# menyifang/MIMO

Measured on NVIDIA H100. Metric: frames/sec @ 512x512x24f, 20 DDIM steps, higher is better.
Workload: dtype fp16

## Files before the change

### mimo_b200/csrc/gemm_wgmma.cu

```cuda
#include <cuda_runtime.h>

#include <cudaTypedefs.h>

#include "../../include/mimo_b200.h"
#include "host_util.h"
#include "ptx.cuh"
#include "wgmma.cuh"

namespace mimo {

constexpr int BM = 128;
constexpr int BK = 64;
constexpr int kGemmThreads = 320;
constexpr int kChunk = 8192;

struct EpiArgs {
  const void* bias;
  const void* rowvec;
  long long rows_per_group;
  long long ld_rowvec;
  float scale;
  int act;
  float* partial;
};

struct ConvGeom {
  int conv;
  int H, W, NI;
  int TW, TH, TN;
  int tiles_w, tiles_h;
  int ctot;
  int c0;
  int kb0, kb1;
  int a_bytes;
  int chunk_bytes;
  int splits;
  int kb_split;
  int ntaps;
  signed char tdx[9], tdy[9];
};

template <int BN, bool kRes>
struct GemmCfg {
  static constexpr int kStageBytes = BM * BK * 2 + BN * BK * 2;
  static constexpr int kNChunk = BN / 32;
  static constexpr int kOutBytes = 2 * kChunk;
  static constexpr int kResSlots = kRes ? 2 : 0;
  static constexpr int kResBytes = kResSlots * kChunk;
  static constexpr int kBarBytes = 512;
  static constexpr int kFixed = kBarBytes + 2048  + kOutBytes + kResBytes;
  static constexpr int kMaxStages = (BN >= 256) ? 4 : (BN >= 160 ? 5 : (BN >= 128 ? 6 : 8));
  static constexpr int kFit = (227 * 1024 - kFixed) / kStageBytes;
  static constexpr int kStages = kFit < kMaxStages ? kFit : kMaxStages;
  static constexpr int kSmemBytes = kStages * kStageBytes + kFixed;
  static_assert(kStages >= 3, "pipeline too shallow");
};

template <int BN, bool kBf16, bool kRes>
__global__ void __launch_bounds__(kGemmThreads, 1)
gemm_wgmma_kernel(const __grid_constant__ CUtensorMap tmA0, const __grid_constant__ CUtensorMap tmA1,
                  const __grid_constant__ CUtensorMap tmB, const __grid_constant__ CUtensorMap tmOut,
                  const __grid_constant__ CUtensorMap tmRes, int M, int N, int num_m_tiles, int num_n_tiles,
                  int num_k_blocks, ConvGeom g, EpiArgs ep) {
  using Cfg = GemmCfg<BN, kRes>;
  using C = Cvt<kBf16>;
  using T = typename C::T;
  constexpr int NCHUNK = Cfg::kNChunk;
  extern __shared__ __align__(1024) uint8_t smem[];
  uint8_t* sOut = smem + Cfg::kStages * Cfg::kStageBytes;
  uint8_t* sRes = sOut + Cfg::kOutBytes;
  uint64_t* bars = reinterpret_cast<uint64_t*>(sRes + Cfg::kResBytes);
  uint64_t* full_bar = bars;
  uint64_t* empty_bar = bars + 8;
  uint64_t* res_full = bars + 16;
  uint64_t* res_empty = bars + 18;
  float* sbias = reinterpret_cast<float*>(reinterpret_cast<uint8_t*>(bars) + Cfg::kBarBytes);

  pdl_launch_dependents();
  const int warp = __shfl_sync(0xffffffffu, threadIdx.x >> 5, 0);
  const int lane = threadIdx.x & 31;
  const int num_tiles = num_m_tiles * num_n_tiles * g.splits;
  auto decode = [&](int tile, int& m_tile, int& n_tile, int& split, int& kb_begin, int& kb_cnt) {
    const int mn = tile / g.splits;
    split = tile - mn * g.splits;
    m_tile = mn / num_n_tiles;
    n_tile = mn - m_tile * num_n_tiles;
    kb_begin = split * g.kb_split;
    kb_cnt = num_k_blocks - kb_begin;
    if (kb_cnt > g.kb_split) kb_cnt = g.kb_split;
  };

  if (warp == 8 && lane == 0) {
    tma_prefetch_desc(&tmA0);
    tma_prefetch_desc(&tmA1);
    tma_prefetch_desc(&tmB);
    tma_prefetch_desc(&tmOut);
    if (kRes) tma_prefetch_desc(&tmRes);
  }
  if (warp == 9 && lane == 0) {
    for (int s = 0; s < Cfg::kStages; ++s) {
      mbar_init(&full_bar[s], 1);
      mbar_init(&empty_bar[s], 8);
    }
    for (int s = 0; s < Cfg::kResSlots; ++s) {
      mbar_init(&res_full[s], 1);
      mbar_init(&res_empty[s], 8);
    }
    fence_mbar_init();
  }
  __syncthreads();
  pdl_wait();

  auto tile_origin = [&](int m_tile, int& x0, int& y0, int& n0) {
    if (g.conv) {
      x0 = (m_tile % g.tiles_w) * g.TW;
      y0 = ((m_tile / g.tiles_w) % g.tiles_h) * g.TH;
      n0 = (m_tile / (g.tiles_w * g.tiles_h)) * g.TN;
    } else {
      x0 = y0 = n0 = 0;
    }
  };

  if (warp == 8) {
    uint32_t stage = 0, phase = 0;
    const int kb_per_tap = g.kb0 + g.kb1;
    for (int tile = blockIdx.x; tile < num_tiles; tile += gridDim.x) {
      int m_tile, n_tile, split, kb_begin, kb_cnt;
      decode(tile, m_tile, n_tile, split, kb_begin, kb_cnt);
      int x0, y0, n0;
      tile_origin(m_tile, x0, y0, n0);
      int tap = kb_per_tap > 0 ? kb_begin / kb_per_tap : 0;
      int rem = kb_begin - tap * kb_per_tap;
      int dx = g.tdx[tap], dy = g.tdy[tap], tap_k = tap * g.ctot;
      for (int kbl = 0, kb = kb_begin; kbl < kb_cnt; ++kbl, ++kb) {
        mbar_wait(&empty_bar[stage], phase ^ 1u);
        uint8_t* sa = smem + stage * Cfg::kStageBytes;
        uint8_t* sb = sa + BM * BK * 2;
        if (elect_one()) {
          if (!g.conv) {
            mbar_expect_tx(&full_bar[stage], BM * BK * 2 + BN * BK * 2);
            if (kb < g.kb0) {
              tma_load_2d(sa, &tmA0, &full_bar[stage], kb * BK, m_tile * BM);
              tma_load_2d(sb, &tmB, &full_bar[stage], kb * BK, n_tile * BN);
            } else {
              tma_load_2d(sa, &tmA1, &full_bar[stage], (kb - g.kb0) * BK, m_tile * BM);
              tma_load_2d(sb, &tmB, &full_bar[stage], g.c0 + (kb - g.kb0) * BK, n_tile * BN);
            }
          } else {
            mbar_expect_tx(&full_bar[stage], g.a_bytes + BN * BK * 2);
            int kcoord;
            if (rem < g.kb0) {
              tma_load_4d(sa, &tmA0, &full_bar[stage], rem * BK, x0 + dx, y0 + dy, n0);
              kcoord = tap_k + rem * BK;
            } else {
              tma_load_4d(sa, &tmA1, &full_bar[stage], (rem - g.kb0) * BK, x0 + dx, y0 + dy, n0);
              kcoord = tap_k + g.c0 + (rem - g.kb0) * BK;
            }
            tma_load_2d(sb, &tmB, &full_bar[stage], kcoord, n_tile * BN);
          }
        }
        __syncwarp();
        if (++rem == kb_per_tap) {
          rem = 0;
          tap_k += g.ctot;
          if (++tap == g.ntaps) tap = 0;
          dx = g.tdx[tap];
          dy = g.tdy[tap];
        }
        if (++stage == Cfg::kStages) {
          stage = 0;
          phase ^= 1u;
        }
      }
    }
  } else if (warp == 9) {
    if constexpr (kRes) {
      uint32_t k = 0;
      for (int tile = blockIdx.x; tile < num_tiles; tile += gridDim.x) {
        const int m_tile = tile / num_n_tiles;
        const int n_tile = tile % num_n_tiles;
        int x0, y0, n0;
        tile_origin(m_tile, x0, y0, n0);
        for (int c = 0; c < NCHUNK; ++c, ++k) {
          const uint32_t slot = k % Cfg::kResSlots;
          mbar_wait(&res_empty[slot], ((k / Cfg::kResSlots) & 1u) ^ 1u);
          if (elect_one()) {
            mbar_expect_tx(&res_full[slot], g.chunk_bytes);
            const int col = n_tile * BN + c * 32;
            if (g.conv)
              tma_load_4d(sRes + slot * kChunk, &tmRes, &res_full[slot], col, x0, y0, n0);
            else
              tma_load_2d(sRes + slot * kChunk, &tmRes, &res_full[slot], col, m_tile * BM);
          }
          __syncwarp();
        }
      }
    }
  } else if (warp < 8) {
    const int wg = warp >> 2;
    const int ct = threadIdx.x;
    const int rbase = wg * 64 + (warp & 3) * 16 + (lane >> 2);
    const int q2 = (lane & 3) * 2;
    const bool issuer = ct == 0;
    const int sw[2] = {(rbase >> 1) & 3, ((rbase + 8) >> 1) & 3};
    const bool do_silu = ep.act == MIMO_ACT_SILU;
    const uint32_t rpg = static_cast<uint32_t>(ep.rows_per_group);
    float acc[BN / 2];
    uint32_t stage = 0, phase = 0, lt = 0, oc = 0, rc = 0;

    for (int tile = blockIdx.x; tile < num_tiles; tile += gridDim.x, ++lt) {
      int m_tile, n_tile, split, kb_begin, kb_cnt;
      decode(tile, m_tile, n_tile, split, kb_begin, kb_cnt);
      int x0, y0, n0;
      tile_origin(m_tile, x0, y0, n0);
      auto tile_groups = [&](int mt, uint32_t& gf, uint32_t& gl) {
        if (!g.conv) {
          const uint32_t m0 = static_cast<uint32_t>(mt) * BM;
          uint32_t m1 = m0 + BM - 1;
          if (m1 > static_cast<uint32_t>(M) - 1) m1 = static_cast<uint32_t>(M) - 1;
          gf = m0 / rpg;
          gl = m1 / rpg;
        } else {
          int tx, ty, tn;
          tile_origin(mt, tx, ty, tn);
          int n1 = tn + g.TN - 1;
          if (n1 > g.NI - 1) n1 = g.NI - 1;
          const uint32_t hw = static_cast<uint32_t>(g.H) * g.W;
          gf = (static_cast<uint32_t>(tn) * hw) / rpg;
          gl = (static_cast<uint32_t>(n1 + 1) * hw - 1) / rpg;
        }
      };
      const int ce = ct;
      auto load_consts = [&](int t) -> float {
        float v = 0.f;
        const int mt = (t / g.splits) / num_n_tiles, nt = (t / g.splits) % num_n_tiles;
        const int col = nt * BN + ce;
        if (ce < BN && col < N) {
          if (ep.bias) v = C::to_f(static_cast<const T*>(ep.bias)[col]);
          if (ep.rowvec) {
            uint32_t gf, gl;
            tile_groups(mt, gf, gl);
            if (gf == gl) v += C::to_f(static_cast<const T*>(ep.rowvec)[static_cast<long long>(gf) * ep.ld_rowvec + col]);
          }
        }
        return ep.act == MIMO_ACT_GEGLU ? v : v * ep.scale;
      };
      float* sb = sbias + (lt & 1u) * 256;
      if (ct < BN) sb[ct] = load_consts(tile);

      uint32_t prev_stage = 0;
      for (int kb = 0; kb < kb_cnt; ++kb) {
        mbar_wait(&full_bar[stage], phase);
        const uint32_t sa = smem_u32(smem + stage * Cfg::kStageBytes);
        const uint64_t da = make_smem_desc_sw128(sa + wg * (64 * 128), 16, 1024);
        const uint64_t db = make_smem_desc_sw128(sa + BM * BK * 2, 16, 1024);
        wgmma_fence();
#pragma unroll
        for (int k = 0; k < BK / 16; ++k) {
          Wgmma<BN, kBf16>::ss(acc, da + 2 * k, db + 2 * k, (kb | k) != 0 ? 1u : 0u);
        }
        wgmma_commit();
        if (kb > 0) {
          wgmma_wait<1>();
          if (lane == 0) mbar_arrive(&empty_bar[prev_stage]);
        }
        prev_stage = stage;
        if (++stage == Cfg::kStages) {
          stage = 0;
          phase ^= 1u;
        }
      }
      wgmma_wait<0>();
      reg_fence(acc);
      if (lane == 0) mbar_arrive(&empty_bar[prev_stage]);

      long long row[2];
      bool row_ok[2];
#pragma unroll
      for (int h = 0; h < 2; ++h) {
        const int r = rbase + 8 * h;
        if (!g.conv) {
          row[h] = static_cast<long long>(m_tile) * BM + r;
          row_ok[h] = row[h] < M;
        } else {
          const int x = r % g.TW, y = (r / g.TW) % g.TH, n = r / (g.TW * g.TH);
          row_ok[h] = (n < g.TN) && (x0 + x < g.W) && (y0 + y < g.H) && (n0 + n < g.NI);
          row[h] = (static_cast<long long>(n0 + n) * g.H + (y0 + y)) * g.W + (x0 + x);
        }
      }
      asm volatile("bar.sync 1, 256;" ::: "memory");

      if (ep.partial) {
#pragma unroll
        for (int h = 0; h < 2; ++h) {
          if (!row_ok[h]) continue;
          float* prow = ep.partial + (static_cast<long long>(split) * M + row[h]) * N;
#pragma unroll
          for (int j = 0; j < BN / 8; ++j) {
            const int col = n_tile * BN + 8 * j + q2;
            if (col < N) *reinterpret_cast<float2*>(prow + col) = make_float2(acc[4 * j + 2 * h], acc[4 * j + 2 * h + 1]);
          }
        }
        continue;
      }

      auto stage_and_store = [&](uint8_t* obuf, int col0) {
        fence_proxy_async_smem();
        if (issuer) tma_store_wait_read0();
        asm volatile("bar.sync 1, 256;" ::: "memory");
        if (issuer) {
          if (g.conv)
            tma_store_4d(&tmOut, obuf, col0, x0, y0, n0);
          else
            tma_store_2d(&tmOut, obuf, col0, m_tile * BM);
          tma_store_commit();
        }
      };

      if (ep.act != MIMO_ACT_GEGLU) {
        const float scale = ep.scale;
        bool rv_uniform = false;
        if (ep.rowvec) {
          uint32_t gf, gl;
          tile_groups(m_tile, gf, gl);
          rv_uniform = gf == gl;
        }
        const bool need_rv = ep.rowvec != nullptr && !rv_uniform;
        const int mode = (!kRes && !do_silu && !need_rv && ep.bias == nullptr && ep.rowvec == nullptr && scale == 1.0f)
                             ? 0 : (need_rv ? 2 : 1);
        const T* rv[2];
#pragma unroll
        for (int h = 0; h < 2; ++h)
          rv[h] = (need_rv && row_ok[h])
                      ? static_cast<const T*>(ep.rowvec) + static_cast<long long>(static_cast<uint32_t>(row[h]) / rpg) * ep.ld_rowvec
                      : nullptr;
#pragma unroll
        for (int c = 0; c < NCHUNK; ++c) {
          uint8_t* obuf = sOut + (oc & 1u) * kChunk;
          ++oc;
          const int col0 = n_tile * BN + c * 32;
          [[maybe_unused]] uint32_t rslot = 0;
          if constexpr (kRes) {
            const uint32_t k = rc++;
            rslot = k % Cfg::kResSlots;
            mbar_wait(&res_full[rslot], (k / Cfg::kResSlots) & 1u);
          }
#pragma unroll
          for (int jj = 0; jj < 4; ++jj) {
            const int j = 4 * c + jj;
            const float2 cst0 = *reinterpret_cast<const float2*>(sb + c * 32 + 8 * jj + q2);
#pragma unroll
            for (int h = 0; h < 2; ++h) {
              const int r = rbase + 8 * h;
              const int off = r * 64 + ((jj ^ sw[h]) << 4) + q2 * 2;
              float f0 = acc[4 * j + 2 * h], f1 = acc[4 * j + 2 * h + 1];
              if (mode != 0) {
                float c0 = cst0.x, c1 = cst0.y;
                if (mode == 2 && rv[h] && col0 + 8 * jj + q2 < N) {
                  const float2 t = C::unpack(__ldg(reinterpret_cast<const unsigned int*>(rv[h] + col0 + 8 * jj + q2)));
                  c0 = fmaf(t.x, scale, c0);
                  c1 = fmaf(t.y, scale, c1);
                }
                f0 = fmaf(f0, scale, c0);
                f1 = fmaf(f1, scale, c1);
              }
              if constexpr (kRes) {
                const float2 t = C::unpack(*reinterpret_cast<const uint32_t*>(sRes + rslot * kChunk + off));
                f0 = fmaf(t.x, scale, f0);
                f1 = fmaf(t.y, scale, f1);
              }
              if (do_silu) {
                f0 = silu_f(f0);
                f1 = silu_f(f1);
              }
              *reinterpret_cast<uint32_t*>(obuf + off) = C::pack(f0, f1);
            }
          }
          if constexpr (kRes) {
            __syncwarp();
            if (lane == 0) mbar_arrive(&res_empty[rslot]);
          }
          stage_and_store(obuf, col0);
        }
      } else {
        constexpr int HALF = BN / 2;
#pragma unroll
        for (int c = 0; c < HALF / 32; ++c) {
          uint8_t* obuf = sOut + (oc & 1u) * kChunk;
          ++oc;
#pragma unroll
          for (int jj = 0; jj < 4; ++jj) {
            const int j = 4 * c + jj, jg = j + HALF / 8;
            const float2 cv = *reinterpret_cast<const float2*>(sb + c * 32 + 8 * jj + q2);
            const float2 cg = *reinterpret_cast<const float2*>(sb + HALF + c * 32 + 8 * jj + q2);
#pragma unroll
            for (int h = 0; h < 2; ++h) {
              const int r = rbase + 8 * h;
              const float f0 = (acc[4 * j + 2 * h] + cv.x) * gelu_erf_fast(acc[4 * jg + 2 * h] + cg.x);
              const float f1 = (acc[4 * j + 2 * h + 1] + cv.y) * gelu_erf_fast(acc[4 * jg + 2 * h + 1] + cg.y);
              *reinterpret_cast<uint32_t*>(obuf + r * 64 + ((jj ^ sw[h]) << 4) + q2 * 2) = C::pack(f0, f1);
            }
          }
          stage_and_store(obuf, n_tile * HALF + c * 32);
        }
      }
    }
    if (issuer) tma_store_wait_all();
  }
}


template <bool kBf16>
__global__ void __launch_bounds__(256)
splitk_reduce_kernel(const float* __restrict__ part, int splits, long long M, int N, const void* __restrict__ bias,
                     const void* __restrict__ rowvec, long long rpg, long long ld_rowvec,
                     const void* __restrict__ res, long long ld_res, float scale, int act, void* __restrict__ out,
                     long long ldo) {
  using C = Cvt<kBf16>;
  using T = typename C::T;
  pdl_launch_dependents();
  pdl_wait();
  const int nv = N >> 3;
  const long long idx = blockIdx.x * static_cast<long long>(blockDim.x) + threadIdx.x;
  if (idx >= M * nv) return;
  const long long row = idx / nv;
  const int col = static_cast<int>(idx - row * nv) * 8;
  float a[8] = {0.f, 0.f, 0.f, 0.f, 0.f, 0.f, 0.f, 0.f};
  for (int s = 0; s < splits; ++s) {
    const float4* p = reinterpret_cast<const float4*>(part + (static_cast<long long>(s) * M + row) * N + col);
    const float4 u0 = p[0], u1 = p[1];
    a[0] += u0.x, a[1] += u0.y, a[2] += u0.z, a[3] += u0.w;
    a[4] += u1.x, a[5] += u1.y, a[6] += u1.z, a[7] += u1.w;
  }
  float cst[8] = {0.f, 0.f, 0.f, 0.f, 0.f, 0.f, 0.f, 0.f};
  auto add_vec = [&](const T* v, float* dst, bool scaled_fma) {
    const uint4 b = *reinterpret_cast<const uint4*>(v);
    const uint32_t w[4] = {b.x, b.y, b.z, b.w};
#pragma unroll
    for (int j = 0; j < 4; ++j) {
      const float2 t = C::unpack(w[j]);
      if (scaled_fma) {
        dst[2 * j] = fmaf(t.x, scale, dst[2 * j]);
        dst[2 * j + 1] = fmaf(t.y, scale, dst[2 * j + 1]);
      } else {
        dst[2 * j] += t.x;
        dst[2 * j + 1] += t.y;
      }
    }
  };
  if (bias) add_vec(static_cast<const T*>(bias) + col, cst, false);
  if (rowvec) add_vec(static_cast<const T*>(rowvec) + (row / rpg) * ld_rowvec + col, cst, false);
  float f[8];
#pragma unroll
  for (int j = 0; j < 8; ++j) f[j] = fmaf(a[j], scale, cst[j] * scale);
  if (res) add_vec(static_cast<const T*>(res) + row * ld_res + col, f, true);
  if (act == MIMO_ACT_SILU) {
#pragma unroll
    for (int j = 0; j < 8; ++j) f[j] = silu_f(f[j]);
  }
  uint4 o;
  o.x = C::pack(f[0], f[1]);
  o.y = C::pack(f[2], f[3]);
  o.z = C::pack(f[4], f[5]);
  o.w = C::pack(f[6], f[7]);
  *reinterpret_cast<uint4*>(static_cast<T*>(out) + row * ldo + col) = o;
}

static int pick_splits(long long tiles, int nkb, long long M, int N, int64_t ws_bytes) {
  if (tiles * 2 > num_sms() || nkb < 32) return 1;
  long long s = num_sms() / tiles;
  if (s > nkb / 16) s = nkb / 16;
  if (s > 16) s = 16;
  while (s > 1 && s * M * N * 4 > ws_bytes) --s;
  return s < 2 ? 1 : static_cast<int>(s);
}

struct Maps {
  CUtensorMap a0, a1, b, out, res;
};

template <int BN, bool kBf16, bool kRes>
static int launch_cfg(const Maps& m, int M, int N, int mt, int nt, int nkb, const ConvGeom& g, const EpiArgs& ep,
                      cudaStream_t st) {
  using Cfg = GemmCfg<BN, kRes>;
  auto kern = gemm_wgmma_kernel<BN, kBf16, kRes>;
  static bool attr_done = false;
  if (!attr_done) {
    cudaError_t e = cudaFuncSetAttribute(kern, cudaFuncAttributeMaxDynamicSharedMemorySize, Cfg::kSmemBytes);
    if (e != cudaSuccess) return set_cuda_error("cudaFuncSetAttribute(gemm)", e);
    attr_done = true;
  }
  const int tiles = mt * nt;
  const int grid = tiles < num_sms() ? tiles : num_sms();
  cudaError_t e = launch_k(kern, dim3(grid), dim3(kGemmThreads), Cfg::kSmemBytes, st, m.a0, m.a1, m.b, m.out, m.res, M, N, mt,
                           nt, nkb, g, ep);
  if (e == cudaSuccess) e = cudaGetLastError();
  if (e != cudaSuccess) return set_cuda_error("gemm launch", e);
  return MIMO_OK;
}

template <bool kBf16>
static int launch_bn(int bn, bool res, const Maps& m, int M, int N, int mt, int nt, int nkb, const ConvGeom& g,
                     const EpiArgs& ep, cudaStream_t st) {
  switch (bn) {
    case 64:
      return res ? launch_cfg<64, kBf16, true>(m, M, N, mt, nt, nkb, g, ep, st)
                 : launch_cfg<64, kBf16, false>(m, M, N, mt, nt, nkb, g, ep, st);
    case 128:
      return res ? launch_cfg<128, kBf16, true>(m, M, N, mt, nt, nkb, g, ep, st)
                 : launch_cfg<128, kBf16, false>(m, M, N, mt, nt, nkb, g, ep, st);
    case 160:
      return res ? launch_cfg<160, kBf16, true>(m, M, N, mt, nt, nkb, g, ep, st)
                 : launch_cfg<160, kBf16, false>(m, M, N, mt, nt, nkb, g, ep, st);
    case 192:
      return res ? launch_cfg<192, kBf16, true>(m, M, N, mt, nt, nkb, g, ep, st)
                 : launch_cfg<192, kBf16, false>(m, M, N, mt, nt, nkb, g, ep, st);
    case 256:
      return res ? launch_cfg<256, kBf16, true>(m, M, N, mt, nt, nkb, g, ep, st)
                 : launch_cfg<256, kBf16, false>(m, M, N, mt, nt, nkb, g, ep, st);
  }
  return set_error(MIMO_ERR_ARG, "gemm: unsupported BN");
}

static int g_force_bn = 0;

int pick_bn(int N, bool geglu, long long m_tiles) {
  if (g_force_bn) return g_force_bn;
  if (geglu) {
    if (N % 256 == 0) return 256;
    if (N % 128 == 0) return 128;
    return 64;
  }
  const int cands[5] = {256, 192, 160, 128, 64};
  int best = 64;
  double best_eff = -1.0;
  for (int i = 0; i < 5; ++i) {
    const int bn = cands[i];
    const int nt = (N + bn - 1) / bn;
    double eff = static_cast<double>(N) / (static_cast<double>(nt) * bn);
    const long long tiles = m_tiles * nt;
    if (tiles < num_sms() && bn > 64) eff *= 0.5 + 0.5 * static_cast<double>(tiles) / num_sms();
    if (eff > best_eff + 1e-9) {
      best_eff = eff;
      best = bn;
    }
  }
  return best;
}

static EpiArgs make_epi(const mimo_epilogue& e, int N) {
  EpiArgs a;
  a.bias = e.bias;
  a.rowvec = e.rowvec;
  a.rows_per_group = e.rows_per_group > 0 ? e.rows_per_group : 1;
  if (a.rows_per_group > 0x7fffffffLL) a.rows_per_group = 0x7fffffffLL;
  a.ld_rowvec = e.ld_rowvec > 0 ? e.ld_rowvec : N;
  a.scale = e.scale;
  a.act = e.act;
  a.partial = nullptr;
  return a;
}

static int g_splitk = 0;

static int launch_reduce(int dtype, const float* part, int splits, long long M, int N, const mimo_epilogue& e, void* out,
                         long long ldo, cudaStream_t st) {
  const long long total = M * (N / 8);
  const unsigned blocks = div_up(total, 256);
  const long long rpg = e.rows_per_group > 0 ? e.rows_per_group : 1;
  const long long ldr = e.ld_rowvec > 0 ? e.ld_rowvec : N;
  cudaError_t err = dtype == MIMO_BF16
                        ? launch_k(splitk_reduce_kernel<true>, dim3(blocks), dim3(256), 0, st, part, splits, M, N, e.bias,
                                   e.rowvec, rpg, ldr, e.residual, static_cast<long long>(e.ld_res), e.scale, e.act, out, ldo)
                        : launch_k(splitk_reduce_kernel<false>, dim3(blocks), dim3(256), 0, st, part, splits, M, N, e.bias,
                                   e.rowvec, rpg, ldr, e.residual, static_cast<long long>(e.ld_res), e.scale, e.act, out, ldo);
  if (err == cudaSuccess) err = cudaGetLastError();
  if (err != cudaSuccess) return set_cuda_error("split-K reduce launch", err);
  return MIMO_OK;
}

}

using namespace mimo;

extern "C" int mimo_debug_splitk(int mode) {
  g_splitk = mode;
  return 0;
}

extern "C" int mimo_debug_force_bn(int bn) {
  g_force_bn = bn;
  return 0;
}

extern "C" int mimo_gemm_geglu_granule(int32_t N) { return pick_bn(N, true, 1 << 20) / 2; }

extern "C" int mimo_gemm(const mimo_gemm_params* p, void* stream) {
  if (!p || !p->a || !p->w || !p->out) return set_error(MIMO_ERR_ARG, "mimo_gemm: null pointer");
  if (p->M <= 0 || p->N <= 0 || p->K <= 0) return set_error(MIMO_ERR_ARG, "mimo_gemm: empty problem");
  if ((p->K % 8) || (p->lda % 8) || (p->ldw % 8) || (p->N % 8) || (p->ldo % 8))
    return set_error(MIMO_ERR_ARG, "mimo_gemm: K, N, lda, ldw, ldo must be multiples of 8");
  if (p->ep.residual && (p->ep.ld_res % 8)) return set_error(MIMO_ERR_ARG, "mimo_gemm: ld_res % 8 != 0");
  const bool geglu = p->ep.act == MIMO_ACT_GEGLU;
  if (geglu && (p->ep.residual || p->ep.rowvec))
    return set_error(MIMO_ERR_ARG, "mimo_gemm: GEGLU takes neither a residual nor a row vector");
  if (int rc = ensure_device()) return rc;
  const int mt = (p->M + BM - 1) / BM;
  const int K1 = p->a1 ? p->K1 : 0;
  if (K1 < 0 || (K1 % 8) || (p->a1 && (p->lda1 % 8))) return set_error(MIMO_ERR_ARG, "mimo_gemm: K1/lda1 % 8 != 0");
  const int kb0 = (p->K + BK - 1) / BK;
  const int kb1 = (K1 + BK - 1) / BK;
  const int nkb = kb0 + kb1;
  int bn = pick_bn(p->N, geglu, mt);
  int splits = 1;
  if (!geglu && g_splitk && p->workspace && !g_force_bn) {
    const int bn_wide = pick_bn(p->N, false, 1 << 20);
    splits = pick_splits(static_cast<long long>(mt) * ((p->N + bn_wide - 1) / bn_wide), nkb, p->M, p->N, p->workspace_bytes);
    if (splits > 1) bn = bn_wide;
  }
  if (geglu && (p->N % bn)) return set_error(MIMO_ERR_ARG, "mimo_gemm: GEGLU needs N % tile == 0");
  const int nt = (p->N + bn - 1) / bn;
  const bool res = p->ep.residual != nullptr && !geglu && splits == 1;

  Maps m;
  const uint64_t adim[2] = {static_cast<uint64_t>(p->K), static_cast<uint64_t>(p->M)};
  const uint64_t astr[1] = {static_cast<uint64_t>(p->lda) * 2};
  const uint32_t abox[2] = {BK, BM};
  if (int rc = encode_tmap(&m.a0, p->dtype, 2, p->a, adim, astr, abox)) return rc;
  m.a1 = m.a0;
  if (K1) {
    const uint64_t a1dim[2] = {static_cast<uint64_t>(K1), static_cast<uint64_t>(p->M)};
    const uint64_t a1str[1] = {static_cast<uint64_t>(p->lda1) * 2};
    if (int rc = encode_tmap(&m.a1, p->dtype, 2, p->a1, a1dim, a1str, abox)) return rc;
  }
  const uint64_t bdim[2] = {static_cast<uint64_t>(p->K + K1), static_cast<uint64_t>(p->N)};
  const uint64_t bstr[1] = {static_cast<uint64_t>(p->ldw) * 2};
  const uint32_t bbox[2] = {BK, static_cast<uint32_t>(bn)};
  if (int rc = encode_tmap(&m.b, p->dtype, 2, p->w, bdim, bstr, bbox)) return rc;
  const int n_out = geglu ? p->N / 2 : p->N;
  const uint64_t odim[2] = {static_cast<uint64_t>(n_out), static_cast<uint64_t>(p->M)};
  const uint64_t ostr[1] = {static_cast<uint64_t>(p->ldo) * 2};
  const uint32_t obox[2] = {32, BM};
  if (int rc = encode_tmap(&m.out, p->dtype, 2, p->out, odim, ostr, obox, 64)) return rc;
  m.res = m.out;
  if (res) {
    const uint64_t rstr[1] = {static_cast<uint64_t>(p->ep.ld_res) * 2};
    if (int rc = encode_tmap(&m.res, p->dtype, 2, p->ep.residual, odim, rstr, obox, 64)) return rc;
  }

  ConvGeom g = {};
  g.kb0 = kb0;
  g.kb1 = kb1;
  g.c0 = p->K;
  g.chunk_bytes = kChunk;
  g.splits = splits;
  g.kb_split = (nkb + splits - 1) / splits;
  EpiArgs ep = make_epi(p->ep, p->N);
  cudaStream_t st = static_cast<cudaStream_t>(stream);
  if (splits > 1) {
    ep.bias = ep.rowvec = nullptr;
    ep.act = MIMO_ACT_NONE;
    ep.scale = 1.0f;
    ep.partial = static_cast<float*>(p->workspace);
  }
  const int rc = p->dtype == MIMO_BF16 ? launch_bn<true>(bn, res, m, p->M, p->N, mt, nt, nkb, g, ep, st)
                                       : launch_bn<false>(bn, res, m, p->M, p->N, mt, nt, nkb, g, ep, st);
  if (rc || splits == 1) return rc;
  return launch_reduce(p->dtype, ep.partial, splits, p->M, p->N, p->ep, p->out, p->ldo, st);
}

static int conv_launch(const mimo_conv3x3_params* p, const void* w, int ntaps, const signed char* tdx,
                       const signed char* tdy, void* out, int sx, int sy, int ow, int oh, void* stream) {
  const int c1 = p->x1 ? p->c1 : 0;
  ConvGeom g = {};
  g.conv = 1;
  g.H = p->h;
  g.W = p->w_;
  g.NI = p->n;
  g.TW = p->w_ < BM ? p->w_ : BM;
  g.TH = BM / g.TW;
  if (g.TH > p->h) g.TH = p->h;
  if (g.TH < 1) g.TH = 1;
  g.TN = BM / (g.TW * g.TH);
  if (g.TN > p->n) g.TN = p->n;
  if (g.TN < 1) g.TN = 1;
  if (g.TN > 1 && g.TH != p->h) g.TN = 1;
  g.tiles_w = (p->w_ + g.TW - 1) / g.TW;
  g.tiles_h = (p->h + g.TH - 1) / g.TH;
  const int tiles_n = (p->n + g.TN - 1) / g.TN;
  g.ctot = p->c0 + c1;
  g.c0 = p->c0;
  g.kb0 = (p->c0 + BK - 1) / BK;
  g.kb1 = (c1 + BK - 1) / BK;
  g.a_bytes = g.TW * g.TH * g.TN * BK * 2;
  g.chunk_bytes = g.TW * g.TH * g.TN * 64;
  g.ntaps = ntaps;
  for (int t = 0; t < 9; ++t) {
    g.tdx[t] = t < ntaps ? tdx[t] : 0;
    g.tdy[t] = t < ntaps ? tdy[t] : 0;
  }
  const int mt = g.tiles_w * g.tiles_h * tiles_n;
  const int nkb = ntaps * (g.kb0 + g.kb1);
  const long long Mrows = static_cast<long long>(p->n) * p->h * p->w_;
  if (Mrows > 0x7fffffffLL) return set_error(MIMO_ERR_ARG, "mimo_conv: too many pixels");
  int bn = pick_bn(p->cout, false, mt);
  int splits = 1;
  if (g_splitk && p->workspace && !g_force_bn && sx == 1 && sy == 1 && p->ldo == p->cout) {
    const int bn_wide = pick_bn(p->cout, false, 1 << 20);
    splits = pick_splits(static_cast<long long>(mt) * ((p->cout + bn_wide - 1) / bn_wide), nkb, Mrows, p->cout,
                         p->workspace_bytes);
    if (splits > 1) bn = bn_wide;
  }
  g.splits = splits;
  g.kb_split = (nkb + splits - 1) / splits;
  const int nt = (p->cout + bn - 1) / bn;
  const bool res = p->ep.residual != nullptr && splits == 1;

  Maps m;
  auto nhwc_map = [&](CUtensorMap* tm, const void* base, int c, long long pitch, uint32_t box_c, int swz, int px,
                      int py, int iw, int ih) {
    const uint64_t dim[4] = {static_cast<uint64_t>(c), static_cast<uint64_t>(p->w_), static_cast<uint64_t>(p->h),
                             static_cast<uint64_t>(p->n)};
    const uint64_t str[3] = {static_cast<uint64_t>(px) * pitch * 2, static_cast<uint64_t>(py) * iw * pitch * 2,
                             static_cast<uint64_t>(ih) * iw * pitch * 2};
    const uint32_t box[4] = {box_c, static_cast<uint32_t>(g.TW), static_cast<uint32_t>(g.TH),
                             static_cast<uint32_t>(g.TN)};
    return encode_tmap(tm, p->dtype, 4, base, dim, str, box, swz);
  };
  if (int rc = nhwc_map(&m.a0, p->x0, p->c0, p->c0, BK, 128, 1, 1, p->w_, p->h)) return rc;
  m.a1 = m.a0;
  if (c1)
    if (int rc = nhwc_map(&m.a1, p->x1, c1, c1, BK, 128, 1, 1, p->w_, p->h)) return rc;
  {
    const uint64_t dim[2] = {static_cast<uint64_t>(ntaps) * g.ctot, static_cast<uint64_t>(p->cout)};
    const uint64_t str[1] = {static_cast<uint64_t>(ntaps) * g.ctot * 2};
    const uint32_t box[2] = {BK, static_cast<uint32_t>(bn)};
    if (int rc = encode_tmap(&m.b, p->dtype, 2, w, dim, str, box)) return rc;
  }
  if (int rc = nhwc_map(&m.out, out, p->cout, p->ldo, 32, 64, sx, sy, ow, oh)) return rc;
  m.res = m.out;
  if (res)
    if (int rc = nhwc_map(&m.res, p->ep.residual, p->cout, p->ep.ld_res, 32, 64, 1, 1, p->w_, p->h)) return rc;

  EpiArgs ep = make_epi(p->ep, p->cout);
  cudaStream_t st = static_cast<cudaStream_t>(stream);
  if (splits > 1) {
    ep.bias = ep.rowvec = nullptr;
    ep.act = MIMO_ACT_NONE;
    ep.scale = 1.0f;
    ep.partial = static_cast<float*>(p->workspace);
  }
  const int rc = p->dtype == MIMO_BF16
                     ? launch_bn<true>(bn, res, m, static_cast<int>(Mrows), p->cout, mt, nt, nkb, g, ep, st)
                     : launch_bn<false>(bn, res, m, static_cast<int>(Mrows), p->cout, mt, nt, nkb, g, ep, st);
  if (rc || splits == 1) return rc;
  return launch_reduce(p->dtype, ep.partial, splits, Mrows, p->cout, p->ep, out, p->ldo, st);
}

static int conv_check(const mimo_conv3x3_params* p, const char* who) {
  if (!p || !p->x0 || !p->w || !p->out) return set_error(MIMO_ERR_ARG, "mimo_conv: null pointer");
  if (p->n <= 0 || p->h <= 0 || p->w_ <= 0 || p->cout <= 0 || p->c0 <= 0)
    return set_error(MIMO_ERR_ARG, "mimo_conv: empty problem");
  const int c1 = p->x1 ? p->c1 : 0;
  if ((p->c0 % 8) || (c1 % 8) || (p->cout % 8) || (p->ldo % 8))
    return set_error(MIMO_ERR_ARG, "mimo_conv: channel counts must be multiples of 8");
  if (p->ep.act == MIMO_ACT_GEGLU) return set_error(MIMO_ERR_ARG, "mimo_conv: GEGLU not supported");
  if (p->ep.residual && (p->ep.ld_res % 8)) return set_error(MIMO_ERR_ARG, "mimo_conv: ld_res % 8 != 0");
  (void)who;
  return ensure_device();
}

extern "C" int mimo_conv3x3(const mimo_conv3x3_params* p, void* stream) {
  if (int rc = conv_check(p, "mimo_conv3x3")) return rc;
  static const signed char dx[9] = {-1, 0, 1, -1, 0, 1, -1, 0, 1};
  static const signed char dy[9] = {-1, -1, -1, 0, 0, 0, 1, 1, 1};
  return conv_launch(p, p->w, 9, dx, dy, p->out, 1, 1, p->w_, p->h, stream);
}

extern "C" int mimo_conv_up2x(const mimo_conv3x3_params* p, void* stream) {
  if (int rc = conv_check(p, "mimo_conv_up2x")) return rc;
  if (p->ep.residual || p->ep.rowvec) return set_error(MIMO_ERR_ARG, "mimo_conv_up2x: bias / activation epilogue only");
  const int ctot = p->c0 + (p->x1 ? p->c1 : 0);
  const size_t esz = 2;
  for (int a = 0; a < 2; ++a)
    for (int b = 0; b < 2; ++b) {
      const signed char dx[4] = {static_cast<signed char>(b - 1), static_cast<signed char>(b),
                                 static_cast<signed char>(b - 1), static_cast<signed char>(b)};
      const signed char dy[4] = {static_cast<signed char>(a - 1), static_cast<signed char>(a - 1),
                                 static_cast<signed char>(a), static_cast<signed char>(a)};
      const char* w = static_cast<const char*>(p->w) + static_cast<size_t>(2 * a + b) * p->cout * 4 * ctot * esz;
      char* out = static_cast<char*>(p->out) + (static_cast<size_t>(a) * 2 * p->w_ + b) * p->ldo * esz;
      if (int rc = conv_launch(p, w, 4, dx, dy, out, 2, 2, 2 * p->w_, 2 * p->h, stream)) return rc;
    }
  return MIMO_OK;
}
```

Measured before the change: 7.992.

## Ping-pong consumer warpgroups for BN=64 GEMM to overlap epilogue with MMA

For BN=64 the kernel now launches two consumer warpgroups that alternate tiles. Each warpgroup computes a full 128-row tile as two 64-row slabs. Named barriers make the two groups take the main loop in turn, so one group's epilogue (bias, activation, residual, TMA store) overlaps the other group's WGMMA loop. Output, residual and bias buffers and residual producer warps are duplicated per owner. The cost is more shared memory, more registers per thread, and more complex barrier and phase bookkeeping.

```diff
diff --git a/mimo_b200/csrc/gemm_wgmma.cu b/mimo_b200/csrc/gemm_wgmma.cu
--- a/mimo_b200/csrc/gemm_wgmma.cu
+++ b/mimo_b200/csrc/gemm_wgmma.cu
@@ -11,7 +11,6 @@
 
 constexpr int BM = 128;
 constexpr int BK = 64;
-constexpr int kGemmThreads = 320;
 constexpr int kChunk = 8192;
 
 struct EpiArgs {
@@ -42,13 +41,18 @@
 
 template <int BN, bool kRes>
 struct GemmCfg {
+  static constexpr bool kPP = BN == 64;
+  static constexpr int kThreads = kPP ? 384 : 320;
+  static constexpr int kSlabs = kPP ? 2 : 1;
+  static constexpr int kEpiThreads = kPP ? 128 : 256;
   static constexpr int kStageBytes = BM * BK * 2 + BN * BK * 2;
   static constexpr int kNChunk = BN / 32;
-  static constexpr int kOutBytes = 2 * kChunk;
+  static constexpr int kOutBytes = (kPP ? 2 : 1) * 2 * kChunk;
   static constexpr int kResSlots = kRes ? 2 : 0;
-  static constexpr int kResBytes = kResSlots * kChunk;
+  static constexpr int kResBytes = (kPP ? 2 : 1) * kResSlots * kChunk;
   static constexpr int kBarBytes = 512;
-  static constexpr int kFixed = kBarBytes + 2048  + kOutBytes + kResBytes;
+  static constexpr int kBiasBytes = (kPP ? 2 : 1) * 2 * 256 * 4;
+  static constexpr int kFixed = kBarBytes + kBiasBytes + kOutBytes + kResBytes;
   static constexpr int kMaxStages = (BN >= 256) ? 4 : (BN >= 160 ? 5 : (BN >= 128 ? 6 : 8));
   static constexpr int kFit = (227 * 1024 - kFixed) / kStageBytes;
   static constexpr int kStages = kFit < kMaxStages ? kFit : kMaxStages;
@@ -57,7 +61,7 @@
 };
 
 template <int BN, bool kBf16, bool kRes>
-__global__ void __launch_bounds__(kGemmThreads, 1)
+__global__ void __launch_bounds__(GemmCfg<BN, kRes>::kThreads, 1)
 gemm_wgmma_kernel(const __grid_constant__ CUtensorMap tmA0, const __grid_constant__ CUtensorMap tmA1,
                   const __grid_constant__ CUtensorMap tmB, const __grid_constant__ CUtensorMap tmOut,
                   const __grid_constant__ CUtensorMap tmRes, int M, int N, int num_m_tiles, int num_n_tiles,
@@ -66,6 +70,9 @@
   using C = Cvt<kBf16>;
   using T = typename C::T;
   constexpr int NCHUNK = Cfg::kNChunk;
+  constexpr bool kPP = Cfg::kPP;
+  constexpr int kOwners = kPP ? 2 : 1;
+  constexpr int kConsumerWarps = kPP ? 4 : 8;
   extern __shared__ __align__(1024) uint8_t smem[];
   uint8_t* sOut = smem + Cfg::kStages * Cfg::kStageBytes;
   uint8_t* sRes = sOut + Cfg::kOutBytes;
@@ -73,7 +80,7 @@
   uint64_t* full_bar = bars;
   uint64_t* empty_bar = bars + 8;
   uint64_t* res_full = bars + 16;
-  uint64_t* res_empty = bars + 18;
+  uint64_t* res_empty = bars + 20;
   float* sbias = reinterpret_cast<float*>(reinterpret_cast<uint8_t*>(bars) + Cfg::kBarBytes);
 
   pdl_launch_dependents();
@@ -100,11 +107,11 @@
   if (warp == 9 && lane == 0) {
     for (int s = 0; s < Cfg::kStages; ++s) {
       mbar_init(&full_bar[s], 1);
-      mbar_init(&empty_bar[s], 8);
+      mbar_init(&empty_bar[s], kConsumerWarps);
     }
-    for (int s = 0; s < Cfg::kResSlots; ++s) {
+    for (int s = 0; s < kOwners * Cfg::kResSlots; ++s) {
       mbar_init(&res_full[s], 1);
-      mbar_init(&res_empty[s], 8);
+      mbar_init(&res_empty[s], kConsumerWarps);
     }
     fence_mbar_init();
   }
@@ -121,96 +128,117 @@
     }
   };
 
-  if (warp == 8) {
-    uint32_t stage = 0, phase = 0;
-    const int kb_per_tap = g.kb0 + g.kb1;
-    for (int tile = blockIdx.x; tile < num_tiles; tile += gridDim.x) {
+  if (warp >= 8) {
+    if (warp == 8) {
+      uint32_t stage = 0, phase = 0;
+      const int kb_per_tap = g.kb0 + g.kb1;
+      for (int tile = blockIdx.x; tile < num_tiles; tile += gridDim.x) {
+        int m_tile, n_tile, split, kb_begin, kb_cnt;
+        decode(tile, m_tile, n_tile, split, kb_begin, kb_cnt);
+        int x0, y0, n0;
+        tile_origin(m_tile, x0, y0, n0);
+        int tap = kb_per_tap > 0 ? kb_begin / kb_per_tap : 0;
+        int rem = kb_begin - tap * kb_per_tap;
+        int dx = g.tdx[tap], dy = g.tdy[tap], tap_k = tap * g.ctot;
+        for (int kbl = 0, kb = kb_begin; kbl < kb_cnt; ++kbl, ++kb) {
+          mbar_wait(&empty_bar[stage], phase ^ 1u);
+          uint8_t* sa = smem + stage * Cfg::kStageBytes;
+          uint8_t* sb = sa + BM * BK * 2;
+          if (elect_one()) {
+            if (!g.conv) {
+              mbar_expect_tx(&full_bar[stage], BM * BK * 2 + BN * BK * 2);
+              if (kb < g.kb0) {
+                tma_load_2d(sa, &tmA0, &full_bar[stage], kb * BK, m_tile * BM);
+                tma_load_2d(sb, &tmB, &full_bar[stage], kb * BK, n_tile * BN);
+              } else {
+                tma_load_2d(sa, &tmA1, &full_bar[stage], (kb - g.kb0) * BK, m_tile * BM);
+                tma_load_2d(sb, &tmB, &full_bar[stage], g.c0 + (kb - g.kb0) * BK, n_tile * BN);
+              }
+            } else {
+              mbar_expect_tx(&full_bar[stage], g.a_bytes + BN * BK * 2);
+              int kcoord;
+              if (rem < g.kb0) {
+                tma_load_4d(sa, &tmA0, &full_bar[stage], rem * BK, x0 + dx, y0 + dy, n0);
+                kcoord = tap_k + rem * BK;
+              } else {
+                tma_load_4d(sa, &tmA1, &full_bar[stage], (rem - g.kb0) * BK, x0 + dx, y0 + dy, n0);
+                kcoord = tap_k + g.c0 + (rem - g.kb0) * BK;
+              }
+              tma_load_2d(sb, &tmB, &full_bar[stage], kcoord, n_tile * BN);
+            }
+          }
+          __syncwarp();
+          if (++rem == kb_per_tap) {
+            rem = 0;
+            tap_k += g.ctot;
+            if (++tap == g.ntaps) tap = 0;
+            dx = g.tdx[tap];
+            dy = g.tdy[tap];
+          }
+          if (++stage == Cfg::kStages) {
+            stage = 0;
+            phase ^= 1u;
+          }
+        }
+      }
+    } else if (warp == 9 || (kPP && warp == 10)) {
+      if constexpr (kRes) {
+        const int owner = warp - 9;
+        uint64_t* rfull = res_full + owner * Cfg::kResSlots;
+        uint64_t* rempty = res_empty + owner * Cfg::kResSlots;
+        uint8_t* rbuf = sRes + owner * Cfg::kResSlots * kChunk;
+        uint32_t k = 0;
+        for (int tile = blockIdx.x + owner * gridDim.x; tile < num_tiles; tile += kOwners * gridDim.x) {
+          const int m_tile = tile / num_n_tiles;
+          const int n_tile = tile % num_n_tiles;
+          int x0, y0, n0;
+          tile_origin(m_tile, x0, y0, n0);
+          for (int c = 0; c < NCHUNK; ++c, ++k) {
+            const uint32_t slot = k % Cfg::kResSlots;
+            mbar_wait(&rempty[slot], ((k / Cfg::kResSlots) & 1u) ^ 1u);
+            if (elect_one()) {
+              mbar_expect_tx(&rfull[slot], g.chunk_bytes);
+              const int col = n_tile * BN + c * 32;
+              if (g.conv)
+                tma_load_4d(rbuf + slot * kChunk, &tmRes, &rfull[slot], col, x0, y0, n0);
+              else
+                tma_load_2d(rbuf + slot * kChunk, &tmRes, &rfull[slot], col, m_tile * BM);
+            }
+            __syncwarp();
+          }
+        }
+      }
+    }
+  } else {
+    constexpr int kSlabs = Cfg::kSlabs;
+    constexpr int kRows = 2 * kSlabs;
+    const int wg = warp >> 2;
+    const int owner = kPP ? wg : 0;
+    const int et = kPP ? (threadIdx.x & 127) : threadIdx.x;
+    const int bar_id = 1 + owner;
+    const int rbase = (kPP ? 0 : wg * 64) + (warp & 3) * 16 + (lane >> 2);
+    auto row_of = [&](int h) { return rbase + 64 * (h >> 1) + 8 * (h & 1); };
+    const int q2 = (lane & 3) * 2;
+    const bool issuer = et == 0;
+    int sw[kRows];
+#pragma unroll
+    for (int h = 0; h < kRows; ++h) sw[h] = (row_of(h) >> 1) & 3;
+    const bool do_silu = ep.act == MIMO_ACT_SILU;
+    const uint32_t rpg = static_cast<uint32_t>(ep.rows_per_group);
+    uint8_t* sOutO = sOut + owner * 2 * kChunk;
+    uint8_t* sResO = sRes + owner * Cfg::kResSlots * kChunk;
+    uint64_t* rfull = res_full + owner * Cfg::kResSlots;
+    uint64_t* rempty = res_empty + owner * Cfg::kResSlots;
+    float acc[kSlabs][BN / 2];
+    uint32_t stage = 0, phase = 0, it = 0, lt = 0, oc = 0, rc = 0;
+
+    for (int tile = blockIdx.x, seq = 0; tile < num_tiles; tile += gridDim.x, ++seq) {
       int m_tile, n_tile, split, kb_begin, kb_cnt;
       decode(tile, m_tile, n_tile, split, kb_begin, kb_cnt);
-      int x0, y0, n0;
-      tile_origin(m_tile, x0, y0, n0);
-      int tap = kb_per_tap > 0 ? kb_begin / kb_per_tap : 0;
-      int rem = kb_begin - tap * kb_per_tap;
-      int dx = g.tdx[tap], dy = g.tdy[tap], tap_k = tap * g.ctot;
-      for (int kbl = 0, kb = kb_begin; kbl < kb_cnt; ++kbl, ++kb) {
-        mbar_wait(&empty_bar[stage], phase ^ 1u);
-        uint8_t* sa = smem + stage * Cfg::kStageBytes;
-        uint8_t* sb = sa + BM * BK * 2;
-        if (elect_one()) {
-          if (!g.conv) {
-            mbar_expect_tx(&full_bar[stage], BM * BK * 2 + BN * BK * 2);
-            if (kb < g.kb0) {
-              tma_load_2d(sa, &tmA0, &full_bar[stage], kb * BK, m_tile * BM);
-              tma_load_2d(sb, &tmB, &full_bar[stage], kb * BK, n_tile * BN);
-            } else {
-              tma_load_2d(sa, &tmA1, &full_bar[stage], (kb - g.kb0) * BK, m_tile * BM);
-              tma_load_2d(sb, &tmB, &full_bar[stage], g.c0 + (kb - g.kb0) * BK, n_tile * BN);
-            }
-          } else {
-            mbar_expect_tx(&full_bar[stage], g.a_bytes + BN * BK * 2);
-            int kcoord;
-            if (rem < g.kb0) {
-              tma_load_4d(sa, &tmA0, &full_bar[stage], rem * BK, x0 + dx, y0 + dy, n0);
-              kcoord = tap_k + rem * BK;
-            } else {
-              tma_load_4d(sa, &tmA1, &full_bar[stage], (rem - g.kb0) * BK, x0 + dx, y0 + dy, n0);
-              kcoord = tap_k + g.c0 + (rem - g.kb0) * BK;
-            }
-            tma_load_2d(sb, &tmB, &full_bar[stage], kcoord, n_tile * BN);
-          }
-        }
-        __syncwarp();
-        if (++rem == kb_per_tap) {
-          rem = 0;
-          tap_k += g.ctot;
-          if (++tap == g.ntaps) tap = 0;
-          dx = g.tdx[tap];
-          dy = g.tdy[tap];
-        }
-        if (++stage == Cfg::kStages) {
-          stage = 0;
-          phase ^= 1u;
-        }
-      }
-    }
-  } else if (warp == 9) {
-    if constexpr (kRes) {
-      uint32_t k = 0;
-      for (int tile = blockIdx.x; tile < num_tiles; tile += gridDim.x) {
-        const int m_tile = tile / num_n_tiles;
-        const int n_tile = tile % num_n_tiles;
-        int x0, y0, n0;
-        tile_origin(m_tile, x0, y0, n0);
-        for (int c = 0; c < NCHUNK; ++c, ++k) {
-          const uint32_t slot = k % Cfg::kResSlots;
-          mbar_wait(&res_empty[slot], ((k / Cfg::kResSlots) & 1u) ^ 1u);
-          if (elect_one()) {
-            mbar_expect_tx(&res_full[slot], g.chunk_bytes);
-            const int col = n_tile * BN + c * 32;
-            if (g.conv)
-              tma_load_4d(sRes + slot * kChunk, &tmRes, &res_full[slot], col, x0, y0, n0);
-            else
-              tma_load_2d(sRes + slot * kChunk, &tmRes, &res_full[slot], col, m_tile * BM);
-          }
-          __syncwarp();
-        }
-      }
-    }
-  } else if (warp < 8) {
-    const int wg = warp >> 2;
-    const int ct = threadIdx.x;
-    const int rbase = wg * 64 + (warp & 3) * 16 + (lane >> 2);
-    const int q2 = (lane & 3) * 2;
-    const bool issuer = ct == 0;
-    const int sw[2] = {(rbase >> 1) & 3, ((rbase + 8) >> 1) & 3};
-    const bool do_silu = ep.act == MIMO_ACT_SILU;
-    const uint32_t rpg = static_cast<uint32_t>(ep.rows_per_group);
-    float acc[BN / 2];
-    uint32_t stage = 0, phase = 0, lt = 0, oc = 0, rc = 0;
-
-    for (int tile = blockIdx.x; tile < num_tiles; tile += gridDim.x, ++lt) {
-      int m_tile, n_tile, split, kb_begin, kb_cnt;
-      decode(tile, m_tile, n_tile, split, kb_begin, kb_cnt);
+      if (kPP && (seq & 1) != wg) {
+        it += kb_cnt;
+        continue;
+      }
       int x0, y0, n0;
       tile_origin(m_tile, x0, y0, n0);
       auto tile_groups = [&](int mt, uint32_t& gf, uint32_t& gl) {
@@ -230,12 +258,11 @@
           gl = (static_cast<uint32_t>(n1 + 1) * hw - 1) / rpg;
         }
       };
-      const int ce = ct;
-      auto load_consts = [&](int t) -> float {
+      auto load_consts = [&](int t, int ce) -> float {
         float v = 0.f;
         const int mt = (t / g.splits) / num_n_tiles, nt = (t / g.splits) % num_n_tiles;
         const int col = nt * BN + ce;
-        if (ce < BN && col < N) {
+        if (col < N) {
           if (ep.bias) v = C::to_f(static_cast<const T*>(ep.bias)[col]);
           if (ep.rowvec) {
             uint32_t gf, gl;
@@ -245,19 +272,27 @@
         }
         return ep.act == MIMO_ACT_GEGLU ? v : v * ep.scale;
       };
-      float* sb = sbias + (lt & 1u) * 256;
-      if (ct < BN) sb[ct] = load_consts(tile);
-
+      float* sb = sbias + owner * 512 + (lt & 1u) * 256;
+      for (int ce = et; ce < BN; ce += Cfg::kEpiThreads) sb[ce] = load_consts(tile, ce);
+
+      if constexpr (kPP) {
+        stage = it % Cfg::kStages;
+        phase = (it / Cfg::kStages) & 1u;
+        if (seq > 0) bar_sync(3 + ((seq - 1) & 1), 256);
+      }
       uint32_t prev_stage = 0;
       for (int kb = 0; kb < kb_cnt; ++kb) {
         mbar_wait(&full_bar[stage], phase);
         const uint32_t sa = smem_u32(smem + stage * Cfg::kStageBytes);
-        const uint64_t da = make_smem_desc_sw128(sa + wg * (64 * 128), 16, 1024);
         const uint64_t db = make_smem_desc_sw128(sa + BM * BK * 2, 16, 1024);
         wgmma_fence();
 #pragma unroll
         for (int k = 0; k < BK / 16; ++k) {
-          Wgmma<BN, kBf16>::ss(acc, da + 2 * k, db + 2 * k, (kb | k) != 0 ? 1u : 0u);
+#pragma unroll
+          for (int s = 0; s < kSlabs; ++s) {
+            const uint64_t da = make_smem_desc_sw128(sa + (kPP ? s : wg) * (64 * 128), 16, 1024);
+            Wgmma<BN, kBf16>::ss(acc[s], da + 2 * k, db + 2 * k, (kb | k) != 0 ? 1u : 0u);
+          }
         }
         wgmma_commit();
         if (kb > 0) {
@@ -271,14 +306,20 @@
         }
       }
       wgmma_wait<0>();
-      reg_fence(acc);
+#pragma unroll
+      for (int s = 0; s < kSlabs; ++s) reg_fence(acc[s]);
       if (lane == 0) mbar_arrive(&empty_bar[prev_stage]);
-
-      long long row[2];
-      bool row_ok[2];
-#pragma unroll
-      for (int h = 0; h < 2; ++h) {
-        const int r = rbase + 8 * h;
+      if constexpr (kPP) {
+        it += kb_cnt;
+        if (tile + static_cast<int>(gridDim.x) < num_tiles) bar_arrive(3 + (seq & 1), 256);
+      }
+      ++lt;
+
+      long long row[kRows];
+      bool row_ok[kRows];
+#pragma unroll
+      for (int h = 0; h < kRows; ++h) {
+        const int r = row_of(h);
         if (!g.conv) {
           row[h] = static_cast<long long>(m_tile) * BM + r;
           row_ok[h] = row[h] < M;
@@ -288,17 +329,18 @@
           row[h] = (static_cast<long long>(n0 + n) * g.H + (y0 + y)) * g.W + (x0 + x);
         }
       }
-      asm volatile("bar.sync 1, 256;" ::: "memory");
+      bar_sync(bar_id, Cfg::kEpiThreads);
 
       if (ep.partial) {
 #pragma unroll
-        for (int h = 0; h < 2; ++h) {
+        for (int h = 0; h < kRows; ++h) {
           if (!row_ok[h]) continue;
           float* prow = ep.partial + (static_cast<long long>(split) * M + row[h]) * N;
 #pragma unroll
           for (int j = 0; j < BN / 8; ++j) {
             const int col = n_tile * BN + 8 * j + q2;
-            if (col < N) *reinterpret_cast<float2*>(prow + col) = make_float2(acc[4 * j + 2 * h], acc[4 * j + 2 * h + 1]);
+            const float* a = acc[h >> 1];
+            if (col < N) *reinterpret_cast<float2*>(prow + col) = make_float2(a[4 * j + 2 * (h & 1)], a[4 * j + 2 * (h & 1) + 1]);
           }
         }
         continue;
@@ -307,7 +349,7 @@
       auto stage_and_store = [&](uint8_t* obuf, int col0) {
         fence_proxy_async_smem();
         if (issuer) tma_store_wait_read0();
-        asm volatile("bar.sync 1, 256;" ::: "memory");
+        bar_sync(bar_id, Cfg::kEpiThreads);
         if (issuer) {
           if (g.conv)
             tma_store_4d(&tmOut, obuf, col0, x0, y0, n0);
@@ -328,32 +370,33 @@
         const bool need_rv = ep.rowvec != nullptr && !rv_uniform;
         const int mode = (!kRes && !do_silu && !need_rv && ep.bias == nullptr && ep.rowvec == nullptr && scale == 1.0f)
                              ? 0 : (need_rv ? 2 : 1);
-        const T* rv[2];
-#pragma unroll
-        for (int h = 0; h < 2; ++h)
+        const T* rv[kRows];
+#pragma unroll
+        for (int h = 0; h < kRows; ++h)
           rv[h] = (need_rv && row_ok[h])
                       ? static_cast<const T*>(ep.rowvec) + static_cast<long long>(static_cast<uint32_t>(row[h]) / rpg) * ep.ld_rowvec
                       : nullptr;
 #pragma unroll
         for (int c = 0; c < NCHUNK; ++c) {
-          uint8_t* obuf = sOut + (oc & 1u) * kChunk;
+          uint8_t* obuf = sOutO + (oc & 1u) * kChunk;
           ++oc;
           const int col0 = n_tile * BN + c * 32;
           [[maybe_unused]] uint32_t rslot = 0;
           if constexpr (kRes) {
             const uint32_t k = rc++;
             rslot = k % Cfg::kResSlots;
-            mbar_wait(&res_full[rslot], (k / Cfg::kResSlots) & 1u);
+            mbar_wait(&rfull[rslot], (k / Cfg::kResSlots) & 1u);
           }
 #pragma unroll
           for (int jj = 0; jj < 4; ++jj) {
             const int j = 4 * c + jj;
             const float2 cst0 = *reinterpret_cast<const float2*>(sb + c * 32 + 8 * jj + q2);
 #pragma unroll
-            for (int h = 0; h < 2; ++h) {
-              const int r = rbase + 8 * h;
+            for (int h = 0; h < kRows; ++h) {
+              const int r = row_of(h);
               const int off = r * 64 + ((jj ^ sw[h]) << 4) + q2 * 2;
-              float f0 = acc[4 * j + 2 * h], f1 = acc[4 * j + 2 * h + 1];
+              const float* a = acc[h >> 1];
+              float f0 = a[4 * j + 2 * (h & 1)], f1 = a[4 * j + 2 * (h & 1) + 1];
               if (mode != 0) {
                 float c0 = cst0.x, c1 = cst0.y;
                 if (mode == 2 && rv[h] && col0 + 8 * jj + q2 < N) {
@@ -365,7 +408,7 @@
                 f1 = fmaf(f1, scale, c1);
               }
               if constexpr (kRes) {
-                const float2 t = C::unpack(*reinterpret_cast<const uint32_t*>(sRes + rslot * kChunk + off));
+                const float2 t = C::unpack(*reinterpret_cast<const uint32_t*>(sResO + rslot * kChunk + off));
                 f0 = fmaf(t.x, scale, f0);
                 f1 = fmaf(t.y, scale, f1);
               }
@@ -378,7 +421,7 @@
           }
           if constexpr (kRes) {
             __syncwarp();
-            if (lane == 0) mbar_arrive(&res_empty[rslot]);
+            if (lane == 0) mbar_arrive(&rempty[rslot]);
           }
           stage_and_store(obuf, col0);
         }
@@ -386,7 +429,7 @@
         constexpr int HALF = BN / 2;
 #pragma unroll
         for (int c = 0; c < HALF / 32; ++c) {
-          uint8_t* obuf = sOut + (oc & 1u) * kChunk;
+          uint8_t* obuf = sOutO + (oc & 1u) * kChunk;
           ++oc;
 #pragma unroll
           for (int jj = 0; jj < 4; ++jj) {
@@ -394,10 +437,12 @@
             const float2 cv = *reinterpret_cast<const float2*>(sb + c * 32 + 8 * jj + q2);
             const float2 cg = *reinterpret_cast<const float2*>(sb + HALF + c * 32 + 8 * jj + q2);
 #pragma unroll
-            for (int h = 0; h < 2; ++h) {
-              const int r = rbase + 8 * h;
-              const float f0 = (acc[4 * j + 2 * h] + cv.x) * gelu_erf_fast(acc[4 * jg + 2 * h] + cg.x);
-              const float f1 = (acc[4 * j + 2 * h + 1] + cv.y) * gelu_erf_fast(acc[4 * jg + 2 * h + 1] + cg.y);
+            for (int h = 0; h < kRows; ++h) {
+              const int r = row_of(h);
+              const float* a = acc[h >> 1];
+              const int e = 2 * (h & 1);
+              const float f0 = (a[4 * j + e] + cv.x) * gelu_erf_fast(a[4 * jg + e] + cg.x);
+              const float f1 = (a[4 * j + e + 1] + cv.y) * gelu_erf_fast(a[4 * jg + e + 1] + cg.y);
               *reinterpret_cast<uint32_t*>(obuf + r * 64 + ((jj ^ sw[h]) << 4) + q2 * 2) = C::pack(f0, f1);
             }
           }
@@ -408,7 +453,6 @@
     if (issuer) tma_store_wait_all();
   }
 }
-
 
 template <bool kBf16>
 __global__ void __launch_bounds__(256)
@@ -492,7 +536,7 @@
   }
   const int tiles = mt * nt;
   const int grid = tiles < num_sms() ? tiles : num_sms();
-  cudaError_t e = launch_k(kern, dim3(grid), dim3(kGemmThreads), Cfg::kSmemBytes, st, m.a0, m.a1, m.b, m.out, m.res, M, N, mt,
+  cudaError_t e = launch_k(kern, dim3(grid), dim3(Cfg::kThreads), Cfg::kSmemBytes, st, m.a0, m.a1, m.b, m.out, m.res, M, N, mt,
                            nt, nkb, g, ep);
   if (e == cudaSuccess) e = cudaGetLastError();
   if (e != cudaSuccess) return set_cuda_error("gemm launch", e);
```

Result: no change. 7.913 (median of 6 runs) (-1.0%).
